# AI-Unicamp/interspeech_ser

Hardware: AMD Instinct MI355X
Metric: utterances/sec (10 s @16 kHz) WavLM-large embed extract (higher is better)
Workload: dtype bf16; 1 GPU; microsoft/wavlm-large embed extract, batch=16 x 10 s @16 kHz per GPU, all 25 hidden states to HBM, mode=bf16; a counted step = 8 such batches (128 utterances per GPU), 2 in flight at a time; batch=16, batches_in_flight=2, frames_per_utt=499, parallelism=utterance-sharded x1, no collective (one process)

## Files before the change

interspeech_ser_amd/csrc/gemm.hip:

```cpp
#include "ser_common.h"
#ifndef SER_GEMM_PP
#define SER_GEMM_PP 27
#endif
#include <stdlib.h>
#include <stdio.h>
#include <atomic>
#include <type_traits>
#ifdef SER_GEMM_DBG
extern "C" { void* ser_gemm_dbg_ptr = nullptr; }
__device__ unsigned long long* ser_gemm_dbg_dev = nullptr;
#endif

typedef const __attribute__((address_space(1))) void* gptr_t;
typedef __attribute__((address_space(3))) void* lptr_t;

__device__ __forceinline__ const char* uniform_ptr(const void* p) {
    const uint64_t v = (uint64_t)p;
    const uint32_t lo = __builtin_amdgcn_readfirstlane((uint32_t)v), hi = __builtin_amdgcn_readfirstlane((uint32_t)(v >> 32));
    return (const char*)(((uint64_t)hi << 32) | lo);
}
template <int BYTES>
__device__ __forceinline__ void dma_lds(const void* ubase, uint32_t voff, uint32_t lds_addr) {
    static_assert(BYTES == 16 || BYTES == 4, "dwordx4 or dword");
    if constexpr (BYTES == 16)
        asm volatile("s_mov_b32 m0, %2\n\tglobal_load_lds_dwordx4 %0, %1" :: "v"(voff), "s"(ubase), "s"(lds_addr) : "memory");
    else
        asm volatile("s_mov_b32 m0, %2\n\tglobal_load_lds_dword %0, %1" :: "v"(voff), "s"(ubase), "s"(lds_addr) : "memory");
}

template <int N>
__device__ __forceinline__ void wait_vmcnt() {
    if constexpr (N == 0) asm volatile("s_waitcnt vmcnt(0)" ::: "memory");
    else if constexpr (N == 1) asm volatile("s_waitcnt vmcnt(1)" ::: "memory");
    else if constexpr (N == 2) asm volatile("s_waitcnt vmcnt(2)" ::: "memory");
    else if constexpr (N == 3) asm volatile("s_waitcnt vmcnt(3)" ::: "memory");
    else if constexpr (N == 4) asm volatile("s_waitcnt vmcnt(4)" ::: "memory");
    else if constexpr (N == 5) asm volatile("s_waitcnt vmcnt(5)" ::: "memory");
    else if constexpr (N == 6) asm volatile("s_waitcnt vmcnt(6)" ::: "memory");
    else if constexpr (N == 7) asm volatile("s_waitcnt vmcnt(7)" ::: "memory");
    else if constexpr (N == 8) asm volatile("s_waitcnt vmcnt(8)" ::: "memory");
    else if constexpr (N == 10) asm volatile("s_waitcnt vmcnt(10)" ::: "memory");
    else if constexpr (N == 12) asm volatile("s_waitcnt vmcnt(12)" ::: "memory");
    else if constexpr (N == 16) asm volatile("s_waitcnt vmcnt(16)" ::: "memory");
    else static_assert(N < 0, "add a case");
}

__device__ __forceinline__ void mfma_scale8(f32x4& acc, const i32x8& a, const i32x8& b, int sa, int sb) {
    asm volatile("v_mfma_scale_f32_16x16x128_f8f6f4 %0, %1, %2, %0, %3, %4 op_sel_hi:[0,0,0]" : "+v"(acc) : "v"(a), "v"(b), "v"(sa), "v"(sb));
}
__device__ __forceinline__ void mfma_scale_drain() {
    asm volatile("s_nop 15\n\ts_nop 15\n\ts_nop 7" ::: "memory");
}

template <int WM, int WN, int TM, int TN, int BK, int ST, int MODE, bool LNEPI, int OM = MODE>
__global__ __launch_bounds__(64 * WM * WN, 2)
void ser_gemm_kernel(const ser_gemm_args p) {
    constexpr int NW = WM * WN, NT = 64 * NW;
    constexpr int BM = WM * TM * 16, BN = WN * TN * 16;
    constexpr int CH = BK / 8;
    constexpr int ROWB = BK * 2;
    constexpr int RPP = 1024 / ROWB;
    constexpr bool M16 = (MODE == SER_MODE_FP16M);
    constexpr int NPL = M16 ? 1 : mode_traits<MODE>::planes;
    constexpr int A_BYTES = BM * ROWB, W_BYTES = BN * ROWB, STAGE = NPL * (A_BYTES + W_BYTES);
    static_assert(!M16 || (BK == 64 && !LNEPI && (BM + BN) % 64 == 0), "FP16M: 64-deep K tiles, dense epilogue");
    constexpr int SCW = BM + BN;
    constexpr int LA = BM / RPP / NW, LW = BN / RPP / NW;
    constexpr int LPT = NPL * (LA + LW);
    constexpr int KS = BK / 32;
    static_assert(BM % (RPP * NW) == 0 && BN % (RPP * NW) == 0, "tile/wave mismatch");
    extern __shared__ __attribute__((aligned(16))) char lds[];

    const int tid = threadIdx.x;
    const int lane = tid & 63;
    const int wave = __builtin_amdgcn_readfirstlane(tid >> 6);
    const int wm = wave / WN, wn = wave % WN;
#ifdef SER_GEMM_DBG
    const unsigned long long dbg_e0 = __builtin_amdgcn_s_memtime();
#endif

    const int ntn = (p.N + BN - 1) / BN;
    const int ntm = (p.M + BM - 1) / BM;
    int bid = blockIdx.x;
    {
        const int nwg = ntm * ntn;
        const int q = nwg >> 3, r = nwg & 7, xcd = bid & 7;
        const int base = (xcd < r) ? xcd * (q + 1) : r * (q + 1) + (xcd - r) * q;
        bid = base + (bid >> 3);
    }
    const int mt = bid / ntn;
    const int nt = bid - mt * ntn;
    const int g = blockIdx.y;
    const int m0 = mt * BM, n0 = nt * BN;

    const unsigned short* Abase = (const unsigned short*)p.A + (int64_t)g * p.a_group_stride;
    const unsigned short* Wbase = (const unsigned short*)p.W + (int64_t)g * p.w_group_stride;

    const int prow = lane / CH, ppos = lane % CH;
    uint32_t aoff[LA], woff[LW];
    const int m0c = m0 < p.M ? m0 : p.M - 1;
    const int64_t arow0 = p.a_rowoff ? (int64_t)p.a_rowoff[m0c] * 8 : (int64_t)m0c * p.lda;
    const char* const Atile = uniform_ptr(Abase + arow0);
    const char* const Wtile = uniform_ptr(Wbase + (int64_t)n0 * p.K);
#pragma unroll
    for (int q = 0; q < LA; ++q) {
        const int R = (q * NW + wave) * RPP + prow;
        const int f = (BK == 64) ? (R & 7) : ((R >> 1) & 3);
        const int c = ppos ^ f;
        int m = m0 + R;
        m = m < p.M ? m : p.M - 1;
        const int64_t arow = p.a_rowoff ? (int64_t)p.a_rowoff[m] * 8 : (int64_t)m * p.lda;
        aoff[q] = (uint32_t)((arow - arow0 + c * 8) * 2);
    }
#pragma unroll
    for (int q = 0; q < LW; ++q) {
        const int R = (q * NW + wave) * RPP + prow;
        const int f = (BK == 64) ? (R & 7) : ((R >> 1) & 3);
        const int c = ppos ^ f;
        int n = n0 + R;
        n = n < p.N ? n : p.N - 1;
        woff[q] = (uint32_t)(((int64_t)(n - n0) * p.K + c * 8) * 2);
    }
    const uint32_t lds0 = __builtin_amdgcn_readfirstlane((uint32_t)(uintptr_t)(__attribute__((address_space(3))) char*)lds);

    const int nk = p.K / BK;
    const int total = M16 ? 2 * nk : nk;
    const int tpc = p.kc ? p.kc / BK : 0x7fffffff;

    unsigned char* const scl = (unsigned char*)(lds + ST * STAGE + (LNEPI ? 0 : BM * 8));
    const int sc_chunk = M16 ? (wave % (SCW / 64)) : 0;
    const bool sc_is_a = sc_chunk * 64 < BM;
    const char* const sc_base = uniform_ptr(sc_is_a ? p.a_scale : p.w_scale);
    const int64_t sc_step = (sc_is_a ? p.a_scale_ld : p.w_scale_ld) * 4;
    uint32_t sc_off = 0;
    if constexpr (M16) {
        const int r = sc_chunk * 64 + lane;
        int i = sc_is_a ? m0 + r : n0 + r - BM;
        const int lim = sc_is_a ? p.M : p.N;
        i = i < lim ? i : lim - 1;
        sc_off = (uint32_t)i * 4u;
    }
    int i_kk = 0, i_cc = 0, i_cj = 0, i_stage = 0;
    const char* is_ua = nullptr; const char* is_uw = nullptr;
    uint32_t is_dstA = 0, is_dstW = 0;
    auto issue_begin = [&]() {
        int64_t koffA = (int64_t)i_cj * p.ldj + (int64_t)i_cc * BK;
        int64_t koffW = (int64_t)i_kk * BK;
        if constexpr (M16) {
            koffA = (int64_t)(i_kk >> 1) * BK + (i_kk & 1) * p.a_plane_stride;
            koffW = (int64_t)(i_kk >> 1) * BK + (i_kk & 1) * p.w_plane_stride;
            if (i_kk & 1) dma_lds<4>(sc_base + (int64_t)(i_kk >> 1) * sc_step, sc_off, lds0 + (uint32_t)(ST * STAGE + (LNEPI ? 0 : BM * 8) + (i_stage * SCW + sc_chunk * 64) * 4));
        }
        is_dstA = lds0 + i_stage * STAGE + wave * 1024;
        is_dstW = is_dstA + NPL * A_BYTES;
        is_ua = Atile + koffA * 2;
        is_uw = Wtile + koffW * 2;
    };
    auto issue_piece = [&](int j) {
        const int pl = j / (LA + LW), q = j % (LA + LW);
        if (q < LA) dma_lds<16>(is_ua + (int64_t)pl * p.a_plane_stride * 2, aoff[q < LA ? q : 0], is_dstA + pl * A_BYTES + q * NW * 1024);
        else dma_lds<16>(is_uw + (int64_t)pl * p.w_plane_stride * 2, woff[q >= LA ? q - LA : 0], is_dstW + pl * W_BYTES + (q - LA) * NW * 1024);
    };
    auto issue_end = [&]() {
        ++i_kk; ++i_cc;
        if (i_cc == tpc) { i_cc = 0; ++i_cj; }
        i_stage = (i_stage + 1 == ST) ? 0 : i_stage + 1;
    };
    auto issue = [&]() {
        issue_begin();
#pragma unroll
        for (int j = 0; j < LPT; ++j) issue_piece(j);
        issue_end();
    };

    f32x4 acc[TN][TM];
#pragma unroll
    for (int a = 0; a < TN; ++a)
#pragma unroll
        for (int b = 0; b < TM; ++b) acc[a][b] = (f32x4){0.f, 0.f, 0.f, 0.f};

    const int frow = lane & 15, fq = lane >> 4;
    const int fsw = (BK == 64) ? (lane & 7) : ((frow >> 1) & 3);
    int offA[KS], offW[KS];
#pragma unroll
    for (int s = 0; s < KS; ++s) {
        const int phys = ((s * 4 + fq) ^ fsw) << 4;
        offA[s] = (wm * TM * 16 + frow) * ROWB + phys;
        offW[s] = NPL * A_BYTES + (wn * TN * 16 + frow) * ROWB + phys;
    }

    constexpr int CPL = TN * 4;
    const int ncol0 = n0 + wn * (TN * 16) + fq * 4;
    const int64_t gcol = (int64_t)g * p.c_group_stride + ncol0;
    float bias[CPL], csum[CPL];
    auto load_cols = [&]() {
#pragma unroll
        for (int j = 0; j < CPL; ++j) { bias[j] = 0.f; csum[j] = 0.f; }
        if (p.bias) {
#pragma unroll
            for (int j4 = 0; j4 < TN; ++j4)
                if (ncol0 + j4 * 16 < p.N) {
                    const f32x4 b = *(const f32x4*)(p.bias + (int64_t)g * p.N + ncol0 + j4 * 16);
                    bias[j4 * 4 + 0] = b[0]; bias[j4 * 4 + 1] = b[1]; bias[j4 * 4 + 2] = b[2]; bias[j4 * 4 + 3] = b[3];
                }
        }
        if (p.ln_colsum) {
#pragma unroll
            for (int j4 = 0; j4 < TN; ++j4)
                if (ncol0 + j4 * 16 < p.N) {
                    const f32x4 b = *(const f32x4*)(p.ln_colsum + ncol0 + j4 * 16);
                    csum[j4 * 4 + 0] = b[0]; csum[j4 * 4 + 1] = b[1]; csum[j4 * 4 + 2] = b[2]; csum[j4 * 4 + 3] = b[3];
                }
        }
    };
    constexpr bool LATE_COLS = M16;
    if constexpr (!LATE_COLS) load_cols();

#pragma unroll
    for (int t = 0; t < ST - 1; ++t)
        if (t < total) issue();

    float* lnst = (float*)(lds + ST * STAGE);
    if (p.ln_stats_in) {
        for (int r = tid; r < BM; r += NT) {
            int m = m0 + r;
            m = m < p.M ? m : p.M - 1;
            const float* ps = p.ln_stats_in + (int64_t)m * p.ln_groups * 2;
            f32x4 pv[16];
#pragma unroll
            for (int u = 0; u < 16; ++u)
                pv[u] = (2 * u < p.ln_groups) ? *(const f32x4*)(ps + 4 * u) : (f32x4){0.f, 0.f, 0.f, 0.f};
            float s1 = 0.f, s2 = 0.f;
#pragma unroll
            for (int u = 0; u < 16; ++u) { s1 += pv[u][0] + pv[u][2]; s2 += pv[u][1] + pv[u][3]; }
            const float invK = 1.0f / (float)p.K;
            const float mu = s1 * invK;
            const float var = fmaxf(s2 * invK - mu * mu, 0.f);
            lnst[2 * r] = mu;
            lnst[2 * r + 1] = rsqrtf(var + p.ln_eps);
            if (p.mean_out && nt == 0 && g == 0 && m0 + r < p.M) p.mean_out[m] = mu + (p.ln_shift ? p.ln_shift[m] : 0.f);
            if (p.lnstat_out && nt == 0 && g == 0 && m0 + r < p.M) *(f32x2*)(p.lnstat_out + 2 * (int64_t)m) = (f32x2){mu, lnst[2 * r + 1]};
        }
        __syncthreads();
    }

#ifdef SER_GEMM_DBG
    const unsigned long long dbg_t0 = __builtin_amdgcn_s_memtime(), dbg_r0 = __builtin_amdgcn_s_memrealtime();
#endif
    constexpr int PP_BIT = NPL == 2 ? (LNEPI ? 16 : 8) : (LNEPI ? 4 : (TM * TN >= 32 ? 1 : 2));
    constexpr bool PP = !M16 && (SER_GEMM_PP & PP_BIT) && NW == 8 && (KS == 2 || NPL == 2);
    constexpr int PH = (NPL == 1 && TM * TN >= 32) ? KS : 1;
    constexpr int SPP = KS / PH;
    constexpr bool PPW = PP && NPL == 2 && KS == 1 && TN >= 8;
    if constexpr (PPW) {
        constexpr int TNH = TN / 2;
        const int late = wave >> 2;
        if (total >= ST - 1) wait_vmcnt<LPT * (ST - 2)>(); else wait_vmcnt<0>();
        __builtin_amdgcn_s_barrier();
        __builtin_amdgcn_sched_barrier(0);
        if (late) __builtin_amdgcn_s_barrier();
        int stage = 0;
        for (int kt = 0; kt < total; ++kt) {
            const bool more = kt + ST - 1 < total;
            if (more) issue();
            const char* sb = lds + stage * STAGE;
            stage = (stage + 1 == ST) ? 0 : stage + 1;
            const bool last = kt + 1 == total;
            bf16x8 ah[TM], al[TM];
#pragma unroll
            for (int ph = 0; ph < 2; ++ph) {
                bf16x8 wh[TNH], wl[TNH];
                if (ph == 0) {
#pragma unroll
                    for (int x = 0; x < TM; ++x) {
                        ah[x] = *(const bf16x8*)(sb + offA[0] + x * 16 * ROWB);
                        al[x] = *(const bf16x8*)(sb + offA[0] + A_BYTES + x * 16 * ROWB);
                    }
                }
#pragma unroll
                for (int x = 0; x < TNH; ++x) {
                    wh[x] = *(const bf16x8*)(sb + offW[0] + (ph * TNH + x) * 16 * ROWB);
                    wl[x] = *(const bf16x8*)(sb + offW[0] + W_BYTES + (ph * TNH + x) * 16 * ROWB);
                }
                asm volatile("s_waitcnt lgkmcnt(0)" ::: "memory");
                if (ph == 1 && late) { if (more) wait_vmcnt<LPT * (ST - 2)>(); else wait_vmcnt<0>(); }
                __builtin_amdgcn_sched_barrier(0);
                __builtin_amdgcn_s_barrier();
                __builtin_amdgcn_sched_barrier(0);
                __builtin_amdgcn_s_setprio(1);
#pragma unroll
                for (int nj = 0; nj < TNH; ++nj)
#pragma unroll
                    for (int mi = 0; mi < TM; ++mi) {
                        const int ni = ph * TNH + nj;
                        acc[ni][mi] = mfma16<MODE>(wl[nj], ah[mi], acc[ni][mi]);
                        acc[ni][mi] = mfma16<MODE>(wh[nj], al[mi], acc[ni][mi]);
                        acc[ni][mi] = mfma16<MODE>(wh[nj], ah[mi], acc[ni][mi]);
                    }
                __builtin_amdgcn_s_setprio(0);
                if (ph == 1 && !late) { if (more) wait_vmcnt<LPT * (ST - 2)>(); else wait_vmcnt<0>(); }
                __builtin_amdgcn_sched_barrier(0);
                if (!(ph == 1 && last && late)) __builtin_amdgcn_s_barrier();
                __builtin_amdgcn_sched_barrier(0);
// ... 125 lines not shown
                const bool stamp = ser_gemm_dbg_dev && blockIdx.x == 40 && lane == 0 && kt >= 8 && kt < 16;
#define SER_STAMP(i) do { __builtin_amdgcn_sched_barrier(0); if (stamp) stp[i] = __builtin_amdgcn_s_memtime(); __builtin_amdgcn_sched_barrier(0); } while (0)
                SER_STAMP(0);
#else
#define SER_STAMP(i) do { } while (0)
#endif
                SER_STAMP(1);
                const char* sb = lds + stage * STAGE;
                const unsigned char* scb = scl + stage * SCW * 4;
                stage = (stage + 1 == ST) ? 0 : stage + 1;
                const bool last = kt + 1 == total;
                constexpr int NPH = EU ? PHE : PHM;
#pragma unroll
                for (int ph = 0; ph < NPH; ++ph) {
                    bf16x8 af[EU ? 1 : SPM][EU ? 1 : TM], wf[EU ? 1 : SPM][EU ? 1 : TN];
                    i32x8 a8[EU ? TMP : 1], w8[EU ? TN : 1];
                    int sa[EU ? TMP : 1], sw[EU ? TN : 1];
                    if constexpr (!EU) h_phase_reads(sb, ph, af, wf);
                    else e_phase_reads(sb, scb, ph, a8, w8, sa, sw);
                    if (ph == 0 && more) { __builtin_amdgcn_sched_barrier(0); issue(); }
                    asm volatile("s_waitcnt lgkmcnt(0)" ::: "memory");
                    if (ph == 0) SER_STAMP(2);
                    if (ph == NPH - 1 && late) wait_landed(more, kt + ST - 1);
                    if (ph == 0) SER_STAMP(3);
                    __builtin_amdgcn_sched_barrier(0);
                    __builtin_amdgcn_s_barrier();
                    __builtin_amdgcn_sched_barrier(0);
                    if (ph == 0) SER_STAMP(4);
                    __builtin_amdgcn_s_setprio(1);
                    if constexpr (!EU) h_phase_mfma(af, wf);
                    else e_phase_mfma(ph, a8, w8, sa, sw);
                    __builtin_amdgcn_s_setprio(0);
                    if (ph == 0) SER_STAMP(5);
                    if (ph == NPH - 1 && !late) wait_landed(more, kt + ST - 1);
                    if (ph == 0) SER_STAMP(6);
                    __builtin_amdgcn_sched_barrier(0);
                    if (!(ph == NPH - 1 && last && late)) __builtin_amdgcn_s_barrier();
                    __builtin_amdgcn_sched_barrier(0);
                    if (ph == 0) SER_STAMP(7);
                }
#ifdef SER_GEMM_DBG
                if (stamp) for (int i = 0; i < 8; ++i) ser_gemm_dbg_dev[262144 + ((wave * 8 + (kt - 8)) * 8 + i)] = stp[i];
#endif
            };
            for (int kt = 0; kt < total; kt += 2) {
                unit(kt, std::false_type{});
                unit(kt + 1, std::true_type{});
            }
        } else {
            int stage = 0;
            auto unit = [&](int kt, auto etag) {
                constexpr bool EU = decltype(etag)::value;
                wait_landed(kt + (ST - 2) < total, kt + ST - 2);
                __builtin_amdgcn_s_barrier();
                if (kt + ST - 1 < total) issue();
                const char* sb = lds + stage * STAGE;
                const unsigned char* scb = scl + stage * SCW * 4;
                stage = (stage + 1 == ST) ? 0 : stage + 1;
#pragma unroll
                for (int ph = 0; ph < (EU ? PHE : PHM); ++ph) {
                    if constexpr (!EU) {
                        bf16x8 af[SPM][TM], wf[SPM][TN];
                        h_phase_reads(sb, ph, af, wf);
                        __builtin_amdgcn_s_setprio(1);
                        h_phase_mfma(af, wf);
                        __builtin_amdgcn_s_setprio(0);
                    } else {
                        i32x8 a8[TMP], w8[TN];
                        int sa[TMP], sw[TN];
                        e_phase_reads(sb, scb, ph, a8, w8, sa, sw);
                        __builtin_amdgcn_s_setprio(1);
                        e_phase_mfma(ph, a8, w8, sa, sw);
                        __builtin_amdgcn_s_setprio(0);
                    }
                }
            };
            for (int kt = 0; kt < total; kt += 2) {
                unit(kt, std::false_type{});
                unit(kt + 1, std::true_type{});
            }
        }
    }
    if constexpr (M16) mfma_scale_drain();
    int c_stage = 0;
    for (int kt = 0; kt < ((PP || M16) ? 0 : total); ++kt) {
        if (kt + (ST - 2) < total) wait_vmcnt<LPT * (ST - 2)>();
        else wait_vmcnt<0>();
        __builtin_amdgcn_s_barrier();
        if (kt + ST - 1 < total) issue();
        const char* sb = lds + c_stage * STAGE;
        c_stage = (c_stage + 1 == ST) ? 0 : c_stage + 1;
        if constexpr (NPL == 1) {
            constexpr bool PIPE = (TM * TN * 4 + KS * (TM + TN) * 4) <= 208;
            bf16x8 af[KS][TM], wf[KS][TN];
            if constexpr (PIPE) {
#pragma unroll
                for (int s = 0; s < KS; ++s) {
#pragma unroll
                    for (int x = 0; x < TM; ++x) af[s][x] = *(const bf16x8*)(sb + offA[s] + x * 16 * ROWB);
#pragma unroll
                    for (int x = 0; x < TN; ++x) wf[s][x] = *(const bf16x8*)(sb + offW[s] + x * 16 * ROWB);
                }
            }
#pragma unroll
            for (int s = 0; s < KS; ++s) {
                if constexpr (!PIPE) {
#pragma unroll
                    for (int x = 0; x < TM; ++x) af[s][x] = *(const bf16x8*)(sb + offA[s] + x * 16 * ROWB);
#pragma unroll
                    for (int x = 0; x < TN; ++x) wf[s][x] = *(const bf16x8*)(sb + offW[s] + x * 16 * ROWB);
                }
                __builtin_amdgcn_s_setprio(1);
#pragma unroll
                for (int ni = 0; ni < TN; ++ni)
#pragma unroll
                    for (int mi = 0; mi < TM; ++mi)
                        acc[ni][mi] = mfma16<MODE>(wf[s][ni], af[s][mi], acc[ni][mi]);
                __builtin_amdgcn_s_setprio(0);
            }
        } else {
#pragma unroll
            for (int s = 0; s < KS; ++s) {
                bf16x8 ah[TM], al[TM], wh[TN], wl[TN];
#pragma unroll
                for (int x = 0; x < TM; ++x) {
                    ah[x] = *(const bf16x8*)(sb + offA[s] + x * 16 * ROWB);
                    al[x] = *(const bf16x8*)(sb + offA[s] + A_BYTES + x * 16 * ROWB);
                }
#pragma unroll
                for (int x = 0; x < TN; ++x) {
                    wh[x] = *(const bf16x8*)(sb + offW[s] + x * 16 * ROWB);
                    wl[x] = *(const bf16x8*)(sb + offW[s] + W_BYTES + x * 16 * ROWB);
                }
                __builtin_amdgcn_s_setprio(1);
#pragma unroll
                for (int ni = 0; ni < TN; ++ni)
#pragma unroll
                    for (int mi = 0; mi < TM; ++mi) {
                        acc[ni][mi] = mfma16<MODE>(wl[ni], ah[mi], acc[ni][mi]);
                        acc[ni][mi] = mfma16<MODE>(wh[ni], al[mi], acc[ni][mi]);
                        acc[ni][mi] = mfma16<MODE>(wh[ni], ah[mi], acc[ni][mi]);
                    }
                __builtin_amdgcn_s_setprio(0);
            }
        }
    }

#ifdef SER_GEMM_DBG
    {
        __builtin_amdgcn_sched_barrier(0);
        const unsigned long long t1 = __builtin_amdgcn_s_memtime(), r1 = __builtin_amdgcn_s_memrealtime();
        unsigned long long* d = ser_gemm_dbg_dev;
        if (d && wave == 0 && lane == 0 && blockIdx.y == 0) {
            d[blockIdx.x * 2] = t1 - dbg_t0; d[blockIdx.x * 2 + 1] = r1 - dbg_r0;
            d[131072 + blockIdx.x * 4] = dbg_t0 - dbg_e0; d[131072 + blockIdx.x * 4 + 1] = t1;
        }
    }
#endif
    if constexpr (LATE_COLS) load_cols();
    float ramax = 0.f;
    if constexpr (LNEPI) {
        __syncthreads();
        float* red = (float*)lds;
        const float invN = 1.0f / (float)p.N;
        float mean[TM], rstd[TM], nmr[TM];
#pragma unroll
        for (int mi = 0; mi < TM; ++mi) {
            float s1 = 0.f, s2 = 0.f;
// ... 153 lines not shown
                    if (ok0 && ncol0 + ni * 16 >= p.f32_col_begin) *(f32x4*)op = o0;
                    if (ok1 && ncol0 + ni * 16 + 16 >= p.f32_col_begin) *(f32x4*)(op + 16) = o1;
                }
                if (p.shift_out) {
#pragma unroll
                    for (int r = 0; r < 8; ++r) v[r] -= cshift;
                }
                if (do_stat && ok0) {
#pragma unroll
                    for (int r = 0; r < 4; ++r) { st1 += v[r]; st2 += v[r] * v[r]; }
                }
                if (do_stat && ok1) {
#pragma unroll
                    for (int r = 4; r < 8; ++r) { st1 += v[r]; st2 += v[r] * v[r]; }
                }
                if (p.out_act) {
                    const int c8 = ni * 16 + ((fq & 1) ? 12 : 0);
                    if constexpr (OM == SER_MODE_FP16M) {
                        store_act8_swap<SER_MODE_FP16>((unsigned short*)p.out_act + orow * p.ldo_act + gcol + c8, 0, ncol0 + c8 < p.N, v);
                        float lo[8], ax = 0.f, al = 0.f;
#pragma unroll
                        for (int r = 0; r < 8; r += 2) {
                            const unsigned h2 = pack_h2(v[r], v[r + 1]);
                            lo[r] = v[r] - h2f((unsigned short)(h2 & 0xffffu));
                            lo[r + 1] = v[r + 1] - h2f((unsigned short)(h2 >> 16));
                            ax = fmaxf(ax, fmaxf(fabsf(v[r]), fabsf(v[r + 1])));
                            al = fmaxf(al, fmaxf(fabsf(lo[r]), fabsf(lo[r + 1])));
                        }
                        if (p.range_flag) range_fold8(ramax, v, ok0, ok1);
                        ax = max_rowquad(ax); al = max_rowquad(al);
                        const unsigned cx = mx_code(ax), cl = mx_code(al);
                        const float ix = mx_inv(cx), il = mx_inv(cl);
                        unsigned q4[4] = {mx_pack4(lo[0] * il, lo[1] * il, lo[2] * il, lo[3] * il), mx_pack4(lo[4] * il, lo[5] * il, lo[6] * il, lo[7] * il),
                                          mx_pack4(v[0] * ix, v[1] * ix, v[2] * ix, v[3] * ix), mx_pack4(v[4] * ix, v[5] * ix, v[6] * ix, v[7] * ix)};
                        transpose_rowquad(q4);
                        const int64_t bcol = gcol - fq * 4 + ni * 16;
                        unsigned char* seg = (unsigned char*)((unsigned short*)p.out_act + p.out_plane_stride) + (orow * p.ldo_act + (bcol & ~(int64_t)63)) * 2;
                        if (ok0) *(u32x4*)(seg + (fq >> 1) * 64 + (bcol & 63) + (fq & 1) * 16) = (u32x4){q4[0], q4[1], q4[2], q4[3]};
                        mcode[(ni >> 1) & 1] = cl | (cx << 16);
                        if (((ni >> 1) & 1) && fq == 0 && ok0)
                            p.out_scale[(bcol >> 6) * p.out_scale_ld + orow] = (mcode[0] & 0xffu) | ((mcode[1] & 0xffu) << 8) | (mcode[0] & 0xff0000u) | ((mcode[1] & 0xff0000u) << 8);
                    } else {
                        store_act8_swap<OM>((unsigned short*)p.out_act + orow * p.ldo_act + gcol + c8, p.out_plane_stride,
                                            ncol0 + c8 < p.N, v);
                        if constexpr (mode_traits<OM>::f16) {
                            if (p.range_flag) range_fold8(ramax, v, ok0, ok1);
                        }
                    }
                }
            }
            if (p.stat_out) {
                st1 += __shfl_xor(st1, 16, 64); st2 += __shfl_xor(st2, 16, 64);
                st1 += __shfl_xor(st1, 32, 64); st2 += __shfl_xor(st2, 32, 64);
                const int cstart = n0 + wn * (TN * 16);
                const int grp = g * ((p.N + 63) >> 6) + (cstart >> 6);
                if (fq == 0 && cstart < p.N && grp < p.stat_groups) {
                    float* d = p.stat_out + ((int64_t)m * p.stat_groups + grp) * 2;
                    d[0] = st1; d[1] = st2;
                    if constexpr (TN * 16 > 64) {
                        if (cstart + 64 < p.N) { d[2] = 0.f; d[3] = 0.f; }
                    }
                }
            }
        }
    }
    if constexpr (mode_traits<OM>::f16) range_report(p.range_flag, ramax);
#ifdef SER_GEMM_DBG
    {
        __builtin_amdgcn_sched_barrier(0);
        asm volatile("s_waitcnt vmcnt(0)" ::: "memory");
        const unsigned long long t2 = __builtin_amdgcn_s_memtime();
        unsigned long long* d = ser_gemm_dbg_dev;
        if (d && wave == 0 && lane == 0 && blockIdx.y == 0) d[131072 + blockIdx.x * 4 + 2] = t2;
    }
#endif
}

#ifdef SER_EXPERIMENTS
#define SER_KNOB(name, dflt) ([] { const char* e_ = getenv(name); return e_ ? atol(e_) : (long)(dflt); }())
#else
#define SER_KNOB(name, dflt) ((long)(dflt))
#endif

enum { CFG_128x128 = 0, CFG_256x128 = 1, CFG_256x256 = 2, CFG_LN512 = 3, CFG_LN512_M64 = 4, CFG_LN512_M32 = 5, CFG_128x64 = 6 };

template <int WM, int WN, int TM, int TN, int BK, int ST, int MODE, bool LNEPI, int OM = MODE>
static hipError_t launch_mode(const ser_gemm_args* a, dim3 grid, dim3 block, int LDS, hipStream_t s) {
    auto k = ser_gemm_kernel<WM, WN, TM, TN, BK, ST, MODE, LNEPI, OM>;
    static std::atomic<bool> ready{false};
    if (LDS > 65536 && !ready.load(std::memory_order_acquire)) {
        hipError_t e = hipFuncSetAttribute((const void*)k, hipFuncAttributeMaxDynamicSharedMemorySize, LDS);
        if (e != hipSuccess) return e;
        ready.store(true, std::memory_order_release);
    }
    hipLaunchKernelGGL(k, grid, block, LDS, s, *a);
    return hipSuccess;
}

template <int WM, int WN, int TM, int TN, int BK, int ST, bool LNEPI, bool X32 = false>
static int launch_cfg(const ser_gemm_args* a, hipStream_t s) {
    constexpr int BM = WM * TM * 16, BN = WN * TN * 16;
    const int npl = (a->mode == SER_MODE_FP32X || a->mode == SER_MODE_FP16X) ? 2 : 1;
    const int LDS = npl * ST * (BM + BN) * BK * 2 + (LNEPI ? 0 : BM * 8)
                  + (a->mode == SER_MODE_FP16M ? ST * (BM + BN) * 4 : 0);
    const int ntm = (a->M + BM - 1) / BM, ntn = (a->N + BN - 1) / BN;
    dim3 grid((unsigned)(ntm * ntn), (unsigned)a->groups, 1), block(64 * WM * WN, 1, 1);
    hipError_t e = hipSuccess;
    if constexpr (X32) {
        if constexpr (!LNEPI) {
            if (a->mode == SER_MODE_FP16X && a->out_mode == SER_MODE_FP16M) {
                if constexpr (BN >= 128)
                    e = launch_mode<WM, WN, TM, TN, BK, ST, SER_MODE_FP16X, LNEPI, SER_MODE_FP16M>(a, grid, block, LDS, s);
                else return ser_fail(-22, "ser_gemm: FP16X -> FP16M output needs a dense tile (N > 64)");
            } else
            if (a->mode == SER_MODE_FP16X && a->out_mode == SER_MODE_FP16)
                e = launch_mode<WM, WN, TM, TN, BK, ST, SER_MODE_FP16X, LNEPI, SER_MODE_FP16>(a, grid, block, LDS, s);
            else if (a->mode == SER_MODE_FP16X)
                e = launch_mode<WM, WN, TM, TN, BK, ST, SER_MODE_FP16X, LNEPI>(a, grid, block, LDS, s);
            else if (a->out_mode == SER_MODE_FP16)
                e = launch_mode<WM, WN, TM, TN, BK, ST, SER_MODE_FP32X, LNEPI, SER_MODE_FP16>(a, grid, block, LDS, s);
            else
                e = launch_mode<WM, WN, TM, TN, BK, ST, SER_MODE_FP32X, LNEPI>(a, grid, block, LDS, s);
        } else {
            if (a->mode == SER_MODE_FP16X)
                e = launch_mode<WM, WN, TM, TN, BK, ST, SER_MODE_FP16X, LNEPI>(a, grid, block, LDS, s);
            else
                e = launch_mode<WM, WN, TM, TN, BK, ST, SER_MODE_FP32X, LNEPI>(a, grid, block, LDS, s);
        }
    } else {
        if (a->mode == SER_MODE_FP16M) {
            if constexpr (!LNEPI && BN >= 128 && BK == 64) {
                if (a->out_mode == SER_MODE_FP16X)
                    e = launch_mode<WM, WN, TM, TN, BK, ST, SER_MODE_FP16M, LNEPI, SER_MODE_FP16X>(a, grid, block, LDS, s);
                else
                    e = launch_mode<WM, WN, TM, TN, BK, ST, SER_MODE_FP16M, LNEPI>(a, grid, block, LDS, s);
            } else return ser_fail(-22, "ser_gemm: FP16M needs a dense tile (N > 64, no LayerNorm epilogue)");
        } else
        if (a->mode == SER_MODE_FP16) {
            if constexpr (!LNEPI && BN >= 128) {
                if (a->out_mode == SER_MODE_FP16X)
                    e = launch_mode<WM, WN, TM, TN, BK, ST, SER_MODE_FP16, LNEPI, SER_MODE_FP16X>(a, grid, block, LDS, s);
                else
                    e = launch_mode<WM, WN, TM, TN, BK, ST, SER_MODE_FP16, LNEPI>(a, grid, block, LDS, s);
            } else {
                if (a->out_mode == SER_MODE_FP16X) return ser_fail(-22, "ser_gemm: FP16 -> FP16X output needs a dense tile (N > 64, no LayerNorm epilogue)");
                e = launch_mode<WM, WN, TM, TN, BK, ST, SER_MODE_FP16, LNEPI>(a, grid, block, LDS, s);
            }
        }
        else e = launch_mode<WM, WN, TM, TN, BK, ST, SER_MODE_BF16, LNEPI>(a, grid, block, LDS, s);
    }
    if (e != hipSuccess) return ser_fail((int)e, "ser_gemm: cannot raise dynamic LDS to %d", LDS);
    return ser_check_launch("ser_gemm");
}

static int pick_cfg(const ser_gemm_args* a) {
    if (a->ln_gamma) {
        static const int force_bm = (int)SER_KNOB("SER_GEMM_LN_BM", 0);
        const int bm = force_bm ? force_bm : (a->M >= 200 * 128 ? 128 : (a->M >= 200 * 64 ? 64 : 32));
        return bm == 128 ? CFG_LN512 : (bm == 64 ? CFG_LN512_M64 : CFG_LN512_M32);
    }
    if (a->tile_cfg > 0) return a->tile_cfg - 1;
#ifdef SER_EXPERIMENTS
    {
        struct Rule { int n, k, cfg; };
        static Rule rules[8];
        static const int nrules = [] {
            const char* e = getenv("SER_GEMM_FORCE");
            int n = 0;
            while (e && *e && n < 8) {
                int a0, a1, a2, used = 0;
                if (sscanf(e, "%d:%d:%d%n", &a0, &a1, &a2, &used) != 3) break;
                rules[n++] = {a0, a1, a2};
                e += used;
                if (*e == ',') ++e;
            }
            return n;
        }();
        for (int i = 0; i < nrules; ++i)
            if (rules[i].n == a->N && rules[i].k == a->K && rules[i].cfg >= 0 && rules[i].cfg <= CFG_256x256) return rules[i].cfg;
    }
#endif
    const long t256x256 = (long)((a->M + 255) / 256) * ((a->N + 255) / 256) * a->groups;
    static const long t256_min = SER_KNOB("SER_GEMM_T256_MIN", 150);
    if (a->N >= 256 && t256x256 >= t256_min) return CFG_256x256;
    static const int n64 = (int)SER_KNOB("SER_GEMM_N64", 1);
    if (n64 && a->N <= 64) return CFG_128x64;
    static const int deepk = (int)SER_KNOB("SER_GEMM_DEEPK_256x128", 1);
    if (deepk && a->groups == 1 && a->K >= 2048 && a->N >= 128 && a->M >= 512) return CFG_256x128;
    return CFG_128x128;
}

extern "C" int ser_gemm(const ser_gemm_args* a, void* stream) {
    if (!a || !a->A || !a->W) return ser_fail(-1, "ser_gemm: null operand");
    if (a->M <= 0 || a->N <= 0 || a->K <= 0) return ser_fail(-2, "ser_gemm: bad shape M=%d N=%d K=%d", a->M, a->N, a->K);
    if (a->K % 64) return ser_fail(-3, "ser_gemm: K=%d must be a multiple of 64", a->K);
    if (a->kc && (a->kc % 64 || a->K % a->kc)) return ser_fail(-4, "ser_gemm: kc=%d must divide K and be a multiple of 64", a->kc);
    if (a->N % 8) return ser_fail(-5, "ser_gemm: N=%d must be a multiple of 8", a->N);
    if (a->mode != SER_MODE_BF16 && a->mode != SER_MODE_FP32X && a->mode != SER_MODE_FP16 && a->mode != SER_MODE_FP16X && a->mode != SER_MODE_FP16M)
        return ser_fail(-6, "ser_gemm: bad mode %d", a->mode);
    if (a->mode == SER_MODE_FP16M) {
        if (!a->a_scale || !a->w_scale || a->a_scale_ld < a->M || a->w_scale_ld < a->N)
            return ser_fail(-23, "ser_gemm: FP16M needs a_scale / w_scale with *_scale_ld >= the row count");
        if (a->a_rowoff || a->kc || a->groups != 1 || a->ln_gamma || (a->lda % 64))
            return ser_fail(-23, "ser_gemm: FP16M takes plain row-major operands (no row map / conv chunks / groups / LayerNorm epilogue), lda %% 64 == 0");
    }
    if (a->out_mode == SER_MODE_FP16M || (a->mode == SER_MODE_FP16M && !a->out_mode && a->out_act)) {
        if (!a->out_scale || (a->N % 64) || (a->ldo_act % 64) || a->groups != 1 || a->ln_gamma)
            return ser_fail(-24, "ser_gemm: an FP16M out_act needs out_scale, N %% 64 == 0, ldo_act %% 64 == 0, groups == 1, no LayerNorm epilogue");
    }
    if (!a->a_rowoff && (a->lda % 8)) return ser_fail(-7, "ser_gemm: lda must be a multiple of 8");
    if (a->groups < 1) return ser_fail(-8, "ser_gemm: groups=%d", a->groups);
    if (!a->out_f32 && !a->out_act) return ser_fail(-9, "ser_gemm: no output");
    if ((a->ldo_f32 % 4) || (a->ldo_act % 4) || (a->ldr % 4) || (a->c_group_stride % 4))
        return ser_fail(-10, "ser_gemm: output/residual pitches must be multiples of 4");
    if (a->ln_gamma) {
        if (!a->ln_beta) return ser_fail(-11, "ser_gemm: ln_gamma without ln_beta");
        if (a->N > 512 || a->groups != 1 || a->residual)
            return ser_fail(-12, "ser_gemm: the LayerNorm epilogue needs N <= 512, groups == 1, no residual");
    }
    if (a->ln_stats_in) {
        if (!a->ln_colsum || a->ln_groups < 2 || a->ln_groups > 32 || (a->ln_groups & 1) || a->ln_gamma)
            return ser_fail(-14, "ser_gemm: deferred LayerNorm needs ln_colsum, an even ln_groups in [2,32] and no fused-LN epilogue");
    }
    if (a->stat_out && (a->ln_gamma || a->stat_groups < a->groups * ((a->N + 63) / 64)))
        return ser_fail(-15, "ser_gemm: stat_out needs stat_groups >= groups*ceil(N/64) and no fused-LN epilogue");
    if (a->shift_out && (!a->stat_out || a->ln_gamma)) return ser_fail(-19, "ser_gemm: shift_out needs stat_out and no fused-LN epilogue");
    if (a->mean_out && !a->ln_stats_in) return ser_fail(-20, "ser_gemm: mean_out needs ln_stats_in");
    if (a->lnstat_out && !a->ln_stats_in) return ser_fail(-20, "ser_gemm: lnstat_out needs ln_stats_in");
    if (a->out_mode && a->out_mode != a->mode && !a->ln_gamma &&
        !((a->mode == SER_MODE_FP32X && a->out_mode == SER_MODE_FP16) || (a->mode == SER_MODE_FP16 && a->out_mode == SER_MODE_FP16X) ||
          (a->mode == SER_MODE_FP16X && a->out_mode == SER_MODE_FP16) || (a->mode == SER_MODE_FP16X && a->out_mode == SER_MODE_FP16M) ||
          (a->mode == SER_MODE_FP16M && a->out_mode == SER_MODE_FP16X)))
        return ser_fail(-21, "ser_gemm: out_mode %d with mode %d (FP32X -> FP16, FP16 <-> FP16X, FP16X <-> FP16M convert)", a->out_mode, a->mode);
    if (a->out_mode && a->out_mode != a->mode && a->ln_gamma)
        return ser_fail(-21, "ser_gemm: out_mode %d with the LayerNorm epilogue", a->out_mode);
    if (a->col_scale_end % 4) return ser_fail(-17, "ser_gemm: col_scale_end must be a multiple of 4");
    if (a->gn_scale && (!a->gn_shift || !a->gn_row_offs || a->gn_B < 1 || a->gn_ld < a->N || (a->gn_ld % 4) || a->groups != 1 ||
                        a->ln_gamma || a->ln_stats_in))
        return ser_fail(-25, "ser_gemm: gn_scale needs gn_shift, gn_row_offs, gn_B >= 1, gn_ld >= N (multiple of 4), groups == 1, "
                             "no LayerNorm epilogue and no deferred LayerNorm");
    if ((a->ldo_act % 8) || (a->c_group_stride % 8)) return ser_fail(-18, "ser_gemm: act pitch / group stride must be multiples of 8");
    if (a->f32_col_begin < 0 || (a->f32_col_begin % 8)) return ser_fail(-16, "ser_gemm: f32_col_begin must be a non-negative multiple of 8");
    if (a->tile_cfg < 0 || a->tile_cfg > 3) return ser_fail(-13, "ser_gemm: tile_cfg=%d (0 auto, 1..3)", a->tile_cfg);
    hipStream_t s = (hipStream_t)stream;
#ifdef SER_GEMM_DBG
    {
        static void* planted = nullptr;
        if (planted != ser_gemm_dbg_ptr) {
            planted = ser_gemm_dbg_ptr;
            (void)hipMemcpyToSymbol(HIP_SYMBOL(ser_gemm_dbg_dev), &planted, sizeof(void*));
        }
    }
#endif
    if (a->mode == SER_MODE_FP32X || a->mode == SER_MODE_FP16X) {
        if (a->ln_gamma) return launch_cfg<2, 4, 4, 8, 32, 2, true, true>(a, s);
        static const int x32_n64 = (int)SER_KNOB("SER_GEMM_N64", 1);
        if (x32_n64 && a->N <= 64) return launch_cfg<4, 1, 2, 4, 32, 2, false, true>(a, s);
        static const long x32_256_min = SER_KNOB("SER_GEMM_X32_256_MIN", 100);
        const long t256x128 = (long)((a->M + 255) / 256) * ((a->N + 127) / 128) * a->groups;
        static const long x32_sq_min = SER_KNOB("SER_GEMM_X32_SQ_MIN", 150);
        const long t256sq = (long)((a->M + 255) / 256) * ((a->N + 255) / 256) * a->groups;
        const long sq_rounds = (t256sq + 255) / 256;
        const bool sq_full = t256sq * 100 >= sq_rounds * 256 * 85;
        if (x32_sq_min > 0 && a->N >= 256 && t256sq >= x32_sq_min && sq_full && a->act == SER_ACT_NONE) return launch_cfg<4, 2, 4, 8, 32, 2, false, true>(a, s);
        if (x32_256_min > 0 && a->N >= 128 && t256x128 >= x32_256_min) return launch_cfg<4, 2, 4, 4, 32, 3, false, true>(a, s);
        return launch_cfg<4, 2, 2, 4, 64, 2, false, true>(a, s);
    }
    if (a->mode == SER_MODE_FP16M) {
        const long t256sq = (long)((a->M + 255) / 256) * ((a->N + 255) / 256);
        const long t256x128 = (long)((a->M + 255) / 256) * ((a->N + 127) / 128);
        static const long m_sq_min = SER_KNOB("SER_GEMM_M16_SQ_MIN", 100), m_256_min = SER_KNOB("SER_GEMM_M16_256_MIN", 100);
        if (a->tile_cfg == 3 || (!a->tile_cfg && a->N >= 256 && t256sq >= m_sq_min)) return launch_cfg<2, 4, 8, 4, 64, 2, false>(a, s);
        if (a->tile_cfg == 2 || (!a->tile_cfg && a->N >= 128 && t256x128 >= m_256_min)) return launch_cfg<4, 2, 4, 4, 64, 3, false>(a, s);
        return launch_cfg<2, 2, 4, 4, 64, 2, false>(a, s);
    }
    switch (pick_cfg(a)) {
        case CFG_LN512:   return launch_cfg<2, 4, 4, 8, 64, 2, true>(a, s);
        case CFG_LN512_M64: return launch_cfg<1, 8, 4, 4, 64, 2, true>(a, s);
        case CFG_LN512_M32: return launch_cfg<1, 4, 2, 8, 64, 2, true>(a, s);
        case CFG_128x64:  return launch_cfg<4, 1, 2, 4, 64, 2, false>(a, s);
        case CFG_256x256: return launch_cfg<2, 4, 8, 4, 64, 2, false>(a, s);
        case CFG_256x128: return launch_cfg<4, 2, 4, 4, 64, 3, false>(a, s);
        default:          return launch_cfg<2, 2, 4, 4, 64, 2, false>(a, s);
    }
}
```

Before: 2011 utterances/s.

## Add resident-window GEMM path for grouped positional conv with shared A rows

```diff
diff --git a/interspeech_ser_amd/csrc/gemm.hip b/interspeech_ser_amd/csrc/gemm.hip
--- a/interspeech_ser_amd/csrc/gemm.hip
+++ b/interspeech_ser_amd/csrc/gemm.hip
@@ -52,7 +52,9 @@
     asm volatile("s_nop 15\n\ts_nop 15\n\ts_nop 7" ::: "memory");
 }
 
-template <int WM, int WN, int TM, int TN, int BK, int ST, int MODE, bool LNEPI, int OM = MODE>
+constexpr int WIN_ROWS = 512;
+constexpr int WIN_ST = 2;
+template <int WM, int WN, int TM, int TN, int BK, int ST, int MODE, bool LNEPI, int OM = MODE, bool WIN = false>
 __global__ __launch_bounds__(64 * WM * WN, 2)
 void ser_gemm_kernel(const ser_gemm_args p) {
     constexpr int NW = WM * WN, NT = 64 * NW;
@@ -69,6 +71,8 @@
     constexpr int LPT = NPL * (LA + LW);
     constexpr int KS = BK / 32;
     static_assert(BM % (RPP * NW) == 0 && BN % (RPP * NW) == 0, "tile/wave mismatch");
+    static_assert(!WIN || (NPL == 1 && !M16 && !LNEPI && BK == 64 && WN == 1 && BN == 64 && ST == 2 && BM + 128 <= WIN_ROWS),
+                  "window form: single-plane 64-column tiles, dense epilogue");
     extern __shared__ __attribute__((aligned(16))) char lds[];
 
     const int tid = threadIdx.x;
@@ -102,8 +106,39 @@
     const int64_t arow0 = p.a_rowoff ? (int64_t)p.a_rowoff[m0c] * 8 : (int64_t)m0c * p.lda;
     const char* const Atile = uniform_ptr(Abase + arow0);
     const char* const Wtile = uniform_ptr(Wbase + (int64_t)n0 * p.K);
+    int wrel[WIN ? TM : 1];
+    bool win_fit = false;
+    int win_need = 0;
+    if constexpr (WIN) {
+        const uint32_t ldj8 = (uint32_t)(p.ldj >> 3);
+        const uint32_t taps = (uint32_t)(p.K / BK);
+        const int ro0 = p.a_rowoff[m0c];
+        bool ok = true;
+#pragma unroll
+        for (int x = 0; x < TM; ++x) {
+            int m = m0 + (wm * TM + x) * 16 + (lane & 15);
+            m = m < p.M ? m : p.M - 1;
+            const uint32_t d = (uint32_t)(p.a_rowoff[m] - ro0);
+            const uint32_t q = d / ldj8;
+            ok = ok && q * ldj8 == d && q <= (uint32_t)WIN_ROWS - taps;
+            wrel[x] = (int)q;
+        }
+        int* const vote = (int*)lds;
+        const bool wave_ok = __ballot(ok) == ~0ull;
+        if (lane == 0) vote[wave] = wave_ok ? 1 : 0;
+        __syncthreads();
+        int all = 1;
+#pragma unroll
+        for (int w = 0; w < NW; ++w) all &= vote[w];
+        __syncthreads();
+        win_fit = __builtin_amdgcn_readfirstlane(all) != 0;
+        const int ml = m0 + BM - 1 < p.M ? m0 + BM - 1 : p.M - 1;
+        win_need = __builtin_amdgcn_readfirstlane((int)((uint32_t)(p.a_rowoff[ml] - ro0) / ldj8 + taps));
+    }
 #pragma unroll
     for (int q = 0; q < LA; ++q) {
+        aoff[q] = 0;
+        if (WIN && win_fit) continue;
         const int R = (q * NW + wave) * RPP + prow;
         const int f = (BK == 64) ? (R & 7) : ((R >> 1) & 3);
         const int c = ppos ^ f;
@@ -216,9 +251,31 @@
     constexpr bool LATE_COLS = M16;
     if constexpr (!LATE_COLS) load_cols();
 
-#pragma unroll
-    for (int t = 0; t < ST - 1; ++t)
-        if (t < total) issue();
+    constexpr int WIN_BYTES = WIN_ROWS * ROWB;
+    int w_tap = 0, w_stage = 0;
+    auto issue_w = [&]() {
+        const char* uw = Wtile + (int64_t)w_tap * BK * 2;
+        const uint32_t dst = lds0 + WIN_BYTES + w_stage * W_BYTES + wave * 1024;
+#pragma unroll
+        for (int q = 0; q < LW; ++q) dma_lds<16>(uw, woff[q], dst + q * NW * 1024);
+        ++w_tap;
+        w_stage = (w_stage + 1 == WIN_ST) ? 0 : w_stage + 1;
+    };
+    if (WIN && win_fit) {
+        const uint32_t rowb = (uint32_t)p.ldj * 2u;
+        for (int q = wave; q * RPP < win_need; q += NW) {
+            const int r = q * RPP + prow;
+            const int rc = r < win_need ? r : win_need - 1;
+            dma_lds<16>(Atile, (uint32_t)rc * rowb + (uint32_t)((ppos ^ (r & 7)) * 16), lds0 + q * 1024);
+        }
+#pragma unroll
+        for (int t = 0; t < WIN_ST - 1; ++t)
+            if (t < total) issue_w();
+    } else {
+#pragma unroll
+        for (int t = 0; t < ST - 1; ++t)
+            if (t < total) issue();
+    }
 
     float* lnst = (float*)(lds + ST * STAGE);
     if (p.ln_stats_in) {
@@ -510,8 +567,42 @@
         }
     }
     if constexpr (M16) mfma_scale_drain();
+    if constexpr (WIN) {
+        if (win_fit) {
+            int r_stage = 0;
+            for (int kt = 0; kt < total; ++kt) {
+                if (kt + (WIN_ST - 2) < total) wait_vmcnt<LW * (WIN_ST - 2)>();
+                else wait_vmcnt<0>();
+                __builtin_amdgcn_s_barrier();
+                if (kt + WIN_ST - 1 < total) issue_w();
+                const char* wb = lds + WIN_BYTES + r_stage * W_BYTES - A_BYTES;
+                r_stage = (r_stage + 1 == WIN_ST) ? 0 : r_stage + 1;
+                bf16x8 af[KS][TM], wf[KS][TN];
+#pragma unroll
+                for (int x = 0; x < TM; ++x) {
+                    const int R = wrel[x] + kt;
+#pragma unroll
+                    for (int s = 0; s < KS; ++s) af[s][x] = *(const bf16x8*)(lds + R * ROWB + (((s * 4 + fq) ^ (R & 7)) << 4));
+                }
+#pragma unroll
+                for (int s = 0; s < KS; ++s)
+#pragma unroll
+                    for (int x = 0; x < TN; ++x) wf[s][x] = *(const bf16x8*)(wb + offW[s] + x * 16 * ROWB);
+#pragma unroll
+                for (int s = 0; s < KS; ++s) {
+                    __builtin_amdgcn_s_setprio(1);
+#pragma unroll
+                    for (int ni = 0; ni < TN; ++ni)
+#pragma unroll
+                        for (int mi = 0; mi < TM; ++mi)
+                            acc[ni][mi] = mfma16<MODE>(wf[s][ni], af[s][mi], acc[ni][mi]);
+                    __builtin_amdgcn_s_setprio(0);
+                }
+            }
+        }
+    }
     int c_stage = 0;
-    for (int kt = 0; kt < ((PP || M16) ? 0 : total); ++kt) {
+    for (int kt = 0; kt < ((PP || M16 || (WIN && win_fit)) ? 0 : total); ++kt) {
         if (kt + (ST - 2) < total) wait_vmcnt<LPT * (ST - 2)>();
         else wait_vmcnt<0>();
         __builtin_amdgcn_s_barrier();
@@ -831,11 +922,12 @@
 #define SER_KNOB(name, dflt) ((long)(dflt))
 #endif
 
-enum { CFG_128x128 = 0, CFG_256x128 = 1, CFG_256x256 = 2, CFG_LN512 = 3, CFG_LN512_M64 = 4, CFG_LN512_M32 = 5, CFG_128x64 = 6 };
-
-template <int WM, int WN, int TM, int TN, int BK, int ST, int MODE, bool LNEPI, int OM = MODE>
+enum { CFG_128x128 = 0, CFG_256x128 = 1, CFG_256x256 = 2, CFG_LN512 = 3, CFG_LN512_M64 = 4, CFG_LN512_M32 = 5, CFG_128x64 = 6,
+       CFG_WIN128x64 = 7, CFG_WIN256x64 = 8 };
+
+template <int WM, int WN, int TM, int TN, int BK, int ST, int MODE, bool LNEPI, int OM = MODE, bool WIN = false>
 static hipError_t launch_mode(const ser_gemm_args* a, dim3 grid, dim3 block, int LDS, hipStream_t s) {
-    auto k = ser_gemm_kernel<WM, WN, TM, TN, BK, ST, MODE, LNEPI, OM>;
+    auto k = ser_gemm_kernel<WM, WN, TM, TN, BK, ST, MODE, LNEPI, OM, WIN>;
     static std::atomic<bool> ready{false};
     if (LDS > 65536 && !ready.load(std::memory_order_acquire)) {
         hipError_t e = hipFuncSetAttribute((const void*)k, hipFuncAttributeMaxDynamicSharedMemorySize, LDS);
@@ -846,15 +938,23 @@
     return hipSuccess;
 }
 
-template <int WM, int WN, int TM, int TN, int BK, int ST, bool LNEPI, bool X32 = false>
+template <int WM, int WN, int TM, int TN, int BK, int ST, bool LNEPI, bool X32 = false, bool WIN = false>
 static int launch_cfg(const ser_gemm_args* a, hipStream_t s) {
     constexpr int BM = WM * TM * 16, BN = WN * TN * 16;
     const int npl = (a->mode == SER_MODE_FP32X || a->mode == SER_MODE_FP16X) ? 2 : 1;
-    const int LDS = npl * ST * (BM + BN) * BK * 2 + (LNEPI ? 0 : BM * 8)
-                  + (a->mode == SER_MODE_FP16M ? ST * (BM + BN) * 4 : 0);
+    int LDS = npl * ST * (BM + BN) * BK * 2 + (LNEPI ? 0 : BM * 8)
+            + (a->mode == SER_MODE_FP16M ? ST * (BM + BN) * 4 : 0);
+    if constexpr (WIN) {
+        constexpr int ring = ST * (BM + BN) * BK * 2, win = WIN_ROWS * BK * 2 + WIN_ST * BN * BK * 2;
+        LDS = ring > win ? ring : win;
+    }
     const int ntm = (a->M + BM - 1) / BM, ntn = (a->N + BN - 1) / BN;
     dim3 grid((unsigned)(ntm * ntn), (unsigned)a->groups, 1), block(64 * WM * WN, 1, 1);
     hipError_t e = hipSuccess;
+    if constexpr (WIN) {
+        if (a->mode == SER_MODE_FP16) e = launch_mode<WM, WN, TM, TN, BK, ST, SER_MODE_FP16, LNEPI, SER_MODE_FP16, true>(a, grid, block, LDS, s);
+        else e = launch_mode<WM, WN, TM, TN, BK, ST, SER_MODE_BF16, LNEPI, SER_MODE_BF16, true>(a, grid, block, LDS, s);
+    } else
     if constexpr (X32) {
         if constexpr (!LNEPI) {
             if (a->mode == SER_MODE_FP16X && a->out_mode == SER_MODE_FP16M) {
@@ -902,12 +1002,20 @@
     return ser_check_launch("ser_gemm");
 }
 
+static bool win_eligible(const ser_gemm_args* a, int bm) {
+    return (a->mode == SER_MODE_BF16 || (a->mode == SER_MODE_FP16 && (!a->out_mode || a->out_mode == SER_MODE_FP16))) &&
+           a->kc == 64 && a->groups > 1 && a->N <= 64 && a->a_rowoff && !a->ln_gamma && !a->ln_stats_in &&
+           a->ldj >= a->kc && a->ldj % 8 == 0 && a->ldj < (1 << 21) &&
+           a->K / a->kc + bm <= WIN_ROWS;
+}
+
 static int pick_cfg(const ser_gemm_args* a) {
     if (a->ln_gamma) {
         static const int force_bm = (int)SER_KNOB("SER_GEMM_LN_BM", 0);
         const int bm = force_bm ? force_bm : (a->M >= 200 * 128 ? 128 : (a->M >= 200 * 64 ? 64 : 32));
         return bm == 128 ? CFG_LN512 : (bm == 64 ? CFG_LN512_M64 : CFG_LN512_M32);
     }
+    if (a->tile_cfg >= 4) return a->tile_cfg == 4 ? CFG_128x64 : (a->tile_cfg == 5 ? CFG_WIN128x64 : CFG_WIN256x64);
     if (a->tile_cfg > 0) return a->tile_cfg - 1;
 #ifdef SER_EXPERIMENTS
     {
@@ -933,7 +1041,14 @@
     static const long t256_min = SER_KNOB("SER_GEMM_T256_MIN", 150);
     if (a->N >= 256 && t256x256 >= t256_min) return CFG_256x256;
     static const int n64 = (int)SER_KNOB("SER_GEMM_N64", 1);
-    if (n64 && a->N <= 64) return CFG_128x64;
+    if (n64 && a->N <= 64) {
+        static const int win = (int)SER_KNOB("SER_GEMM_WIN", 1);
+        static const long win256_min = SER_KNOB("SER_GEMM_WIN256_MIN", 384);
+        const long t256 = (long)((a->M + 255) / 256) * a->groups;
+        if (win && t256 >= win256_min && win_eligible(a, 256)) return CFG_WIN256x64;
+        if (win && win_eligible(a, 128)) return CFG_WIN128x64;
+        return CFG_128x64;
+    }
     static const int deepk = (int)SER_KNOB("SER_GEMM_DEEPK_256x128", 1);
     if (deepk && a->groups == 1 && a->K >= 2048 && a->N >= 128 && a->M >= 512) return CFG_256x128;
     return CFG_128x128;
@@ -990,7 +1105,14 @@
                              "no LayerNorm epilogue and no deferred LayerNorm");
     if ((a->ldo_act % 8) || (a->c_group_stride % 8)) return ser_fail(-18, "ser_gemm: act pitch / group stride must be multiples of 8");
     if (a->f32_col_begin < 0 || (a->f32_col_begin % 8)) return ser_fail(-16, "ser_gemm: f32_col_begin must be a non-negative multiple of 8");
-    if (a->tile_cfg < 0 || a->tile_cfg > 3) return ser_fail(-13, "ser_gemm: tile_cfg=%d (0 auto, 1..3)", a->tile_cfg);
+    if (a->tile_cfg < 0 || a->tile_cfg > 6) return ser_fail(-13, "ser_gemm: tile_cfg=%d (0 auto, 1..6)", a->tile_cfg);
+    if (a->tile_cfg >= 4 && (a->mode != SER_MODE_BF16 && a->mode != SER_MODE_FP16))
+        return ser_fail(-13, "ser_gemm: tile_cfg=%d is a single-plane tile (mode %d)", a->tile_cfg, a->mode);
+    if (a->tile_cfg >= 4 && (a->ln_gamma || (a->mode == SER_MODE_FP16 && a->out_mode == SER_MODE_FP16X)))
+        return ser_fail(-13, "ser_gemm: tile_cfg=%d takes no LayerNorm epilogue and no FP16X output", a->tile_cfg);
+    if (a->tile_cfg >= 5 && !win_eligible(a, a->tile_cfg == 5 ? 128 : 256))
+        return ser_fail(-13, "ser_gemm: tile_cfg=%d (resident window) needs a grouped conv map: kc == 64, groups > 1, N <= 64, a_rowoff, "
+                             "ldj %% 8 == 0, K / kc + tile rows <= %d, no LayerNorm", a->tile_cfg, WIN_ROWS);
     hipStream_t s = (hipStream_t)stream;
 #ifdef SER_GEMM_DBG
     {
@@ -1028,6 +1150,8 @@
         case CFG_LN512_M64: return launch_cfg<1, 8, 4, 4, 64, 2, true>(a, s);
         case CFG_LN512_M32: return launch_cfg<1, 4, 2, 8, 64, 2, true>(a, s);
         case CFG_128x64:  return launch_cfg<4, 1, 2, 4, 64, 2, false>(a, s);
+        case CFG_WIN128x64: return launch_cfg<4, 1, 2, 4, 64, 2, false, false, true>(a, s);
+        case CFG_WIN256x64: return launch_cfg<4, 1, 4, 4, 64, 2, false, false, true>(a, s);
         case CFG_256x256: return launch_cfg<2, 4, 8, 4, 64, 2, false>(a, s);
         case CFG_256x128: return launch_cfg<4, 2, 4, 4, 64, 3, false>(a, s);
         default:          return launch_cfg<2, 2, 4, 4, 64, 2, false>(a, s);
```

New measurement: 2017 utterances/s, median of 6. Within noise of the previous version (+0.3%).
